# Enigmatisms/Distributed-Machine-Learning-Experiment-Document

Hardware: AMD Instinct MI355X
Metric: samples/sec (whole node) for task3 DDP CNN at 1/2/4/8 MI355X (higher is better)
Workload: dtype bf16; 1 GPU; model=resnet18, global_batch=1024, per_gpu_batch=1024, image_size=224, parallelism=dp1, optimizer=SGD(momentum=0.9), fused flat, ddp=none (dp1: no communication), backend=native, fused_step=False, hip_graph=False, stream_priority=high, sampler=MySampler(partition)

## Files before the change

csrc/stem_fused.hip:

```cpp
#include <type_traits>

#include "common.h"
#include "igemm_common.h"
#include "kernels.h"

namespace dm {

namespace {

constexpr int SCO = 64;
constexpr int SKP = 176;
constexpr int SKH = 192;
constexpr int RING = 13;

typedef short s4v __attribute__((ext_vector_type(4)));
typedef unsigned int nt4 __attribute__((ext_vector_type(4)));
typedef unsigned int nt2 __attribute__((ext_vector_type(2)));
__device__ __forceinline__ s4v tr4(const unsigned char* p) {
  return __builtin_amdgcn_ds_read_tr16_b64_v4i16((__attribute__((address_space(3))) s4v*)p);
}

struct StemGeo {
  int Hin, Win, Hout, Wout, PH, PW;
  int ROWB;
  int SP;
};

struct RawUnit {
  uint4 w;
};

__device__ __forceinline__ void lds_barrier() {
  asm volatile("s_waitcnt lgkmcnt(0)\n\ts_barrier" ::: "memory");
}

__device__ __forceinline__ int ring_of(int iy) { return (iy + 13 * 8) % RING; }

template <int NT, int RU>
struct RawMap {
  int r[RU], k[RU];
  unsigned valid;
  float sc[RU][4], bi[RU][4];
  __device__ __forceinline__ void init(int t, int Win, const float (&nsc)[3], const float (&nbi)[3]) {
    const int upr = 3 * Win / 4;
#pragma unroll
    for (int u = 0; u < RU; ++u) {
      const int e = t + NT * u;
      r[u] = e < 4 * upr ? e / upr : -1;
      k[u] = e - (e / upr) * upr;
#pragma unroll
      for (int j = 0; j < 4; ++j) {
        const int c = (k[u] + j) % 3;
        sc[u][j] = c == 0 ? nsc[0] : c == 1 ? nsc[1] : nsc[2];
        bi[u][j] = c == 0 ? nbi[0] : c == 1 ? nbi[1] : nbi[2];
      }
    }
  }
  template <int DT>
  __device__ __forceinline__ void load(RawUnit (&ru)[RU], const void* img, long long rowbase, int Hin,
                                       int Win, int iy0, int nrows) {
    valid = 0;
#pragma unroll
    for (int u = 0; u < RU; ++u) {
      const int iy = iy0 + r[u];
      const bool ok = r[u] >= 0 && r[u] < nrows && iy >= 0 && iy < Hin;
      valid |= ok ? 1u << u : 0u;
      const int iyc = min(max(iy, 0), Hin - 1);
      const long long off = rowbase + (long long)iyc * Win * 3 + 4LL * (r[u] >= 0 ? k[u] : 0);
      if (DT == 0) {
        ru[u].w = *reinterpret_cast<const uint4*>(reinterpret_cast<const float*>(img) + off);
      } else if (DT == 1) {
        const uint2 w = *reinterpret_cast<const uint2*>(reinterpret_cast<const bf16_t*>(img) + off);
        ru[u].w = make_uint4(w.x, w.y, 0, 0);
      } else {
        ru[u].w = make_uint4(*reinterpret_cast<const uint32_t*>(reinterpret_cast<const uint8_t*>(img) + off), 0, 0, 0);
      }
    }
  }
  template <int DT>
  __device__ __forceinline__ void store(const RawUnit (&ru)[RU], bf16_t* S, int SP, int nrows) const {
#pragma unroll
    for (int u = 0; u < RU; ++u) {
      if (r[u] < 0 || r[u] >= nrows) continue;
      float x[4];
      const uint4 w = ru[u].w;
      if (DT == 0) {
        x[0] = __uint_as_float(w.x); x[1] = __uint_as_float(w.y);
        x[2] = __uint_as_float(w.z); x[3] = __uint_as_float(w.w);
      } else if (DT == 1) {
        x[0] = __uint_as_float(w.x << 16); x[1] = __uint_as_float(w.x & 0xffff0000u);
        x[2] = __uint_as_float(w.y << 16); x[3] = __uint_as_float(w.y & 0xffff0000u);
      } else {
        x[0] = (float)(w.x & 0xff); x[1] = (float)((w.x >> 8) & 0xff);
        x[2] = (float)((w.x >> 16) & 0xff); x[3] = (float)(w.x >> 24);
      }
      const bool ok = (valid >> u) & 1;
#pragma unroll
      for (int j = 0; j < 4; ++j) x[j] = ok ? fmaf(x[j], sc[u][j], bi[u][j]) : 0.f;
      bf16_t* p = S + r[u] * SP + 4 * k[u] + 9;
      p[0] = f2bf(x[0]);
      *reinterpret_cast<uint32_t*>(p + 1) = pack_bf2(x[1], x[2]);
      p[3] = f2bf(x[3]);
    }
  }
};

struct EMap {
  bool act;
  int soff, eoff;
  int part;
  __device__ __forceinline__ void init(int t, int Wout) {
    act = t < 3 * Wout;
    const int ox = t / 3;
    part = t - 3 * ox;
    soff = 6 * ox + 8 * part;
    eoff = 48 * ox + 16 * part;
  }
  __device__ __forceinline__ void build(unsigned char* E, const bf16_t* S, const StemGeo& G, int iy0,
                                        int nrows, int srow0) const {
    if (!act) return;
    if (nrows == 4) build_n<4>(E, S, G, iy0, srow0);
    else if (nrows == 2) build_n<2>(E, S, G, iy0, srow0);
    else for (int q = 0; q < nrows; ++q) build_n<1>(E, S, G, iy0 + q, srow0 + q);
  }
  template <int NR>
  __device__ __forceinline__ void build_n(unsigned char* E, const bf16_t* S, const StemGeo& G,
                                          int iy0, int srow0) const {
    uint32_t w[NR][4];
#pragma unroll
    for (int q = 0; q < NR; ++q) {
      const int sr = min(max(srow0 + q, 0), 3);
      const uint32_t* sp = reinterpret_cast<const uint32_t*>(S + sr * G.SP + soff);
#pragma unroll
      for (int j = 0; j < 4; ++j) w[q][j] = sp[j];
    }
#pragma unroll
    for (int q = 0; q < NR; ++q) {
      const int iy = iy0 + q;
      const bool in = iy >= 0 && iy < G.Hin;
      uint4 v = make_uint4(in ? w[q][0] : 0u, in ? w[q][1] : 0u, in ? w[q][2] : 0u, in ? w[q][3] : 0u);
      if (part == 2) {
        v.z = in ? (v.z & 0xffffu) | 0x3f800000u : 0u;
        v.w = 0;
      }
      *reinterpret_cast<uint4*>(E + ring_of(iy) * G.ROWB + eoff) = v;
    }
  }
};

__host__ __device__ constexpr unsigned wcode(int kh, int kw) { return (unsigned)((2 - kh) << 2 | (2 - kw)); }

__device__ __forceinline__ uint32_t mono2(uint32_t w) {
  const uint32_t s = (w >> 15) & 0x00010001u;
  return w ^ (s * 0x7fffu);
}

__device__ __forceinline__ int yoff(int slot, int px, int c8, int Wout) {
  return ((slot * Wout + px) * 8 + (c8 ^ ((((px >> 1) & 1) << 2) | ((px >> 2) & 3)))) * 16;
}

template <int PF>
__device__ __forceinline__ f32x16 conv_tile(const bf16x8 (&wa)[11], const unsigned char* E,
                                            const int (&rowoff)[7], int pxoff, bool hh) {
  f32x16 acc;
#pragma unroll
  for (int r = 0; r < 16; ++r) acc[r] = 0.f;
  bf16x8 bq[11];
#pragma unroll
  for (int s = 0; s < 11 + PF; ++s) {
    if (s < 11) {
      const int j0 = 2 * s, j1 = 2 * s + 1;
      const int k0 = j0 / 3 > 6 ? 6 : j0 / 3, k1 = j1 / 3 > 6 ? 6 : j1 / 3;
      const int a0 = rowoff[k0] + 16 * (j0 % 3), a1 = rowoff[k1] + 16 * (j1 % 3);
      bq[s] = *reinterpret_cast<const bf16x8*>(E + (hh ? a1 : a0) + pxoff);
    }
    if (s >= PF) acc = __builtin_amdgcn_mfma_f32_32x32x16_bf16(wa[s - PF], bq[s - PF], acc, 0, 0, 0);
  }
  return acc;
}

__device__ __forceinline__ void ring_rows(int (&ro)[7], int iy0, int ROWB) {
  const int r0 = ring_of(iy0);
// ... 355 lines not shown

template <int W>
__device__ __forceinline__ void gram_slot(f32x16 (&acc)[5], const unsigned char* T,
                                          const unsigned char* E, const StemGeo& G, int i,
                                          int slot, int t0, int t1, int lane) {
  constexpr WavePlan P = kPlans[W];
  const int g = lane >> 4, h = g >> 1, i16 = lane & 15, q = i16 >> 2, p = i16 & 3;
  const int oy = 2 * i + slot;
  int boff[4];
#pragma unroll
  for (int b = 0; b < P.nb; ++b) {
    const int k = 32 * P.blk[b] + 16 * (g & 1) + 4 * p;
    int ky = k / 24;
    const int kk = k - 24 * ky;
    if (ky > 6) ky = 6;
    boff[b] = ring_of(2 * oy - 3 + ky) * G.ROWB + (4 * h + q) * 48 + 2 * kk;
  }
  int ta = 0, ta8 = 0;
  if (P.tcb >= 0) {
    const int c8 = 4 * P.tcb + 2 * (g & 1) + (p >> 1);
    ta = yoff(slot, 4 * h + q, c8, G.Wout) + 8 * (p & 1);
    ta8 = yoff(slot, 4 * h + q + 8, c8, G.Wout) + 8 * (p & 1);
  }
  auto load = [&](BwdFrags& F, int t) {
    const int mo = 16 * t;
#pragma unroll
    for (int b = 0; b < P.nb; ++b) {
      const s4v v0 = tr4(E + boff[b] + mo * 48), v1 = tr4(E + boff[b] + (mo + 8) * 48);
      F.xf[b] = (bf16x8){v0[0], v0[1], v0[2], v0[3], v1[0], v1[1], v1[2], v1[3]};
    }
    if (P.tcb >= 0) {
      const s4v v0 = tr4(T + ta + mo * 128), v1 = tr4(T + ta8 + mo * 128);
      F.tf = (bf16x8){v0[0], v0[1], v0[2], v0[3], v1[0], v1[1], v1[2], v1[3]};
    }
  };
  auto mma = [&](const BwdFrags& F) {
#pragma unroll
    for (int j = 0; j < P.nt; ++j)
      acc[j] = __builtin_amdgcn_mfma_f32_32x32x16_bf16(P.kind[j] ? F.tf : F.xf[P.x[j]], F.xf[P.y[j]],
                                                       acc[j], 0, 0, 0);
  };
  for (int t = t0; t < t1; ++t) {
    BwdFrags f;
    load(f, t);
    mma(f);
  }
}

template <int W>
__device__ __forceinline__ void gram_store(const f32x16 (&acc)[5], float* dslab, float* gslab,
                                           int lane) {
  constexpr WavePlan P = kPlans[W];
#pragma unroll
  for (int j = 0; j < P.nt; ++j)
#pragma unroll
    for (int r = 0; r < 16; ++r) {
      const int row = (r & 3) + 8 * (r >> 2) + 4 * (lane >> 5);
      const int col = 32 * P.blk[P.y[j]] + (lane & 31);
      if (P.kind[j])
        dslab[(long long)blockIdx.x * SCO * SKH + (32 * P.tcb + row) * SKH + col] = acc[j][r];
      else
        gslab[(long long)blockIdx.x * GK * GK + (32 * P.blk[P.x[j]] + row) * GK + col] = acc[j][r];
    }
}

template <int W>
__device__ __forceinline__ void gram_zero(f32x16 (&acc)[5]) {
#pragma unroll
  for (int j = 0; j < 5; ++j)
#pragma unroll
    for (int r = 0; r < 16; ++r) acc[j][r] = 0.f;
}

struct StemBwdArgs2 {
  const void* img;
  const long long* idx;
  float nsc[3], nbi[3];
  const bf16_t* wk;
  const bf16_t* pdy;
  const uint8_t* code4;
  float* dslab;
  float* gslab;
  int N, nimg;
  int split;
  StemGeo G;
};

constexpr int PRING = 3;
constexpr int BNT = 1024;
constexpr int BMW = 8;
constexpr int BVT = BNT - 64 * BMW;

template <int DT>
__global__ void __launch_bounds__(BNT, 1) stem_bwd_kernel(StemBwdArgs2 a) {
  extern __shared__ __attribute__((aligned(16))) unsigned char smem[];
  const StemGeo G = a.G;
  const int TB = 2 * G.Wout * 128;
  unsigned char* E = smem;
  unsigned char* T = E + RING * G.ROWB;
  bf16_t* S = reinterpret_cast<bf16_t*>(T + 2 * TB);
  const int PRB = G.PW * SCO;
  bf16_t* Pg = S + 4 * G.SP;
  uint8_t* Pc = reinterpret_cast<uint8_t*>(Pg + PRING * PRB);
  const int tid = threadIdx.x, lane = tid & 63, wid = tid >> 6;
  {
    const int tot16 = (RING * G.ROWB + 2 * TB + 4 * G.SP * 2) / 16;
    for (int e = tid; e < tot16; e += BNT) reinterpret_cast<uint4*>(smem)[e] = make_uint4(0, 0, 0, 0);
  }
  const int nimg = a.N > (int)blockIdx.x ? (a.N - 1 - (int)blockIdx.x) / (int)gridDim.x + 1 : 0;
  const int SPI = G.PH + 2;
  const int nsteps = nimg * SPI;
  auto img_of = [&](int q) { return (int)blockIdx.x + q * (int)gridDim.x; };
  auto img_base = [&](int q) -> long long {
    long long row = a.idx ? a.idx[img_of(q)] : (long long)img_of(q);
    row = row < 0 ? 0 : row >= a.nimg ? a.nimg - 1 : row;
    return row * G.Hin * G.Win * 3;
  };
  if (wid < BMW) {
    f32x16 acc[5];
    gram_zero<0>(acc);
    __syncthreads();
    EMap em;
    em.init(tid, G.Wout);
    auto run = [&](auto wtag) {
      constexpr int W = decltype(wtag)::value;
      for (int st = 0; st <= nsteps; ++st) {
        lds_barrier();
        const int ps = st - 1;
        const int pk = ps >= 0 ? ps % SPI : -1;
        const bool work = ps >= 0 && pk >= 2;
        const unsigned char* Tt = T + (ps & 1) * TB;
        const int nt = G.Wout >> 4, split = min(a.split, 2 * nt);
        if (work) {
          gram_slot<W>(acc, Tt, E, G, pk - 2, 0, 0, min(split, nt), lane);
          if (split > nt) gram_slot<W>(acc, Tt, E, G, pk - 2, 1, 0, split - nt, lane);
        }
        lds_barrier();
        if (work) {
          if (split < nt) gram_slot<W>(acc, Tt, E, G, pk - 2, 0, split, nt, lane);
          gram_slot<W>(acc, Tt, E, G, pk - 2, 1, max(split - nt, 0), nt, lane);
        }
        if (st < nsteps) {
          const int kk = st % SPI;
          if (kk == 1) em.build(E, S, G, -3, 5, -3);
          else if (kk >= 2) em.build(E, S, G, 4 * (kk - 2) + 2, 4, 0);
        }
      }
      gram_store<W>(acc, a.dslab, a.gslab, lane);
    };
    switch (wid) {
      case 0: run(std::integral_constant<int, 0>{}); break;
      case 1: run(std::integral_constant<int, 1>{}); break;
      case 2: run(std::integral_constant<int, 2>{}); break;
      case 3: run(std::integral_constant<int, 3>{}); break;
      case 4: run(std::integral_constant<int, 4>{}); break;
      case 5: run(std::integral_constant<int, 5>{}); break;
      case 6: run(std::integral_constant<int, 6>{}); break;
      default: run(std::integral_constant<int, 7>{}); break;
    }
    return;
  }
  const int vt = tid - 64 * BMW;
  RawMap<BVT, FRU> rm;
  rm.init(vt, G.Win, a.nsc, a.nbi);
  RawUnit ru[FRU];
  const bool pl = vt < G.PW * 8;
  uint4 pg_r;
  uint32_t pc_r;
  bool p_ok = false;
  auto pload = [&](int q, int r) {
    p_ok = pl && r < G.PH;
    const int rc = min(r, G.PH - 1), vc = pl ? vt : 0;
    const long long o = (((long long)img_of(min(q, nimg - 1)) * G.PH + rc) * G.PW) * SCO + vc * 8;
    pg_r = *reinterpret_cast<const uint4*>(a.pdy + o);
    pc_r = *reinterpret_cast<const uint32_t*>(a.code4 + o / 2);
  };
  auto pstore = [&](int r) {
    if (!pl) return;
    const int sl = r % PRING;
    *reinterpret_cast<uint4*>(Pg + sl * PRB + vt * 8) = p_ok ? pg_r : make_uint4(0, 0, 0, 0);
    *reinterpret_cast<uint32_t*>(Pc + (sl * PRB + vt * 8) / 2) = p_ok ? pc_r : 0xffffffffu;
  };
  const int qb = vt >> 3, qc = vt & 7, c0 = qc * 8;
  __syncthreads();
  const bool colok = qb + 1 < G.PW;
  const int ocol0 = qb * SCO + c0, ocol1 = (colok ? qb + 1 : qb) * SCO + c0;
  int toff[4];
#pragma unroll
  for (int pp = 0; pp < 4; ++pp) toff[pp] = yoff(pp >> 1, 2 * qb + (pp & 1), qc, G.Wout);
  uint2 gres[4];
  auto gquad = [&](uint2 (&res)[4], int i, int hf) {
    uint2 qg[4];
    uint32_t qi[4];
    const int sl0 = i % PRING, sl1 = sl0 + 1 == PRING ? 0 : sl0 + 1;
    const bool rowok = i + 1 < G.PH;
#pragma unroll
    for (int w = 0; w < 4; ++w) {
      const int wa = w >> 1, wb = w & 1;
      const int o = (wa ? sl1 : sl0) * PRB + (wb ? ocol1 : ocol0);
      qg[w] = *reinterpret_cast<const uint2*>(Pg + o + 4 * hf);
      const uint32_t c = *reinterpret_cast<const uint16_t*>(Pc + o / 2 + 2 * hf);
      qi[w] = ((wa && !rowok) || (wb && !colok)) ? 0xffffu : c;
    }
#pragma unroll
    for (int pp = 0; pp < 4; ++pp) {
      const int ddy = pp >> 1, ddx = pp & 1;
      float d[4] = {0.f, 0.f, 0.f, 0.f};
#pragma unroll
      for (int w = 0; w < 4; ++w) {
        const int wa = w >> 1, wb = w & 1;
        if ((wa && !ddy) || (wb && !ddx)) continue;
        const uint32_t gw[2] = {qg[w].x, qg[w].y};
        const unsigned code = wcode(ddy ? (wa ? 0 : 2) : 1, ddx ? (wb ? 0 : 2) : 1);
#pragma unroll
        for (int j = 0; j < 4; ++j) {
          const uint32_t g = gw[j >> 1];
          const float gf = __uint_as_float((j & 1) ? (g & 0xffff0000u) : (g << 16));
          d[j] += (qi[w] & (15u << (4 * j))) == (code << (4 * j)) ? gf : 0.f;
        }
      }
      res[pp] = make_uint2(pack_bf2(d[0], d[1]), pack_bf2(d[2], d[3]));
    }
  };


  long long bcur = nimg > 0 ? img_base(0) : 0, bnext = nimg > 1 ? img_base(1) : 0;
  int bq = 0;
  auto base = [&](int qq) {
    if (qq != bq) {
      bcur = bnext;
      bq = qq;
      bnext = qq + 1 < nimg ? img_base(qq + 1) : 0;
    }
    return bcur;
  };
  for (int st = 0; st <= nsteps; ++st) {
    const int q = st / SPI, kk = st - q * SPI;
    lds_barrier();
    if (st < nsteps) {
      if (kk == 0) {
        pload(q, 0);
        pstore(0);
        pload(q, 1);
        pstore(1);
        pload(q, 2);
      } else if (kk == 1) {
        rm.store<DT>(ru, S, G.SP, 2);
      } else {
        const int i = kk - 2;
        pstore(i + 2);
        pload(q, i + 3);
        rm.store<DT>(ru, S, G.SP, 4);
        if (pl) gquad(gres, i, 0);
      }
    }
    lds_barrier();
    if (st < nsteps) {
      if (kk == 0) {
        rm.load<DT>(ru, a.img, base(q), G.Hin, G.Win, 0, 2);
      } else if (kk == 1) {
        rm.load<DT>(ru, a.img, base(q), G.Hin, G.Win, 2, 4);
      } else {
        const int i = kk - 2;
        if (pl) {
          uint2 r1[4];
          gquad(r1, i, 1);
          unsigned char* Tt = T + (st & 1) * TB;
#pragma unroll
          for (int pp = 0; pp < 4; ++pp)
            *reinterpret_cast<uint4*>(Tt + toff[pp]) = make_uint4(gres[pp].x, gres[pp].y, r1[pp].x, r1[pp].y);
        }
        if (i + 1 < G.PH) rm.load<DT>(ru, a.img, base(q), G.Hin, G.Win, 4 * i + 6, 4);
      }
    }
  }
}

__global__ void __launch_bounds__(256) stem_slab_reduce_kernel(const float* __restrict__ dslab,
                                                               const float* __restrict__ gslab,
                                                               int GD, float* __restrict__ dsum,
                                                               float* __restrict__ gsum) {
  const int e = blockIdx.x * 256 + threadIdx.x;
  const int nd = SCO * SKH, ng = GK * GK;
  if (e >= nd + ng) return;
  const float* src = e < nd ? dslab + e : gslab + (e - nd);
  const long long stride = e < nd ? nd : ng;
  float s4[4] = {0.f, 0.f, 0.f, 0.f};
  int gi = 0;
  for (; gi + 4 <= GD; gi += 4)
#pragma unroll
    for (int u = 0; u < 4; ++u) s4[u] += src[(long long)(gi + u) * stride];
  for (; gi < GD; ++gi) s4[0] += src[(long long)gi * stride];
  const float v = (s4[0] + s4[1]) + (s4[2] + s4[3]);
  if (e < nd) dsum[e] = v;
  else gsum[e - nd] = v;
}

__global__ void __launch_bounds__(256) stem_wcombine_kernel(const float* __restrict__ dsum,
                                                            const float* __restrict__ gsum,
                                                            const bf16_t* __restrict__ wk,
                                                            const float* __restrict__ coef,
                                                            float* __restrict__ dw, float beta) {
  __shared__ float wrow[SKP];
  const int co = blockIdx.x, t = threadIdx.x;
  for (int k = t; k < SKP; k += 256) wrow[k] = bf2f(wk[co * SKP + k]);
  __syncthreads();
  if (t >= 147) return;
  const int ky = t / 21, rem = t - 21 * ky, kx = rem / 3, c = rem - 3 * kx;
  const int k = ky * 24 + kx * 3 + c;
  float wg = 0.f;
  for (int j = 0; j < SKP; ++j) {
    const float gv = j <= k ? gsum[j * GK + k] : gsum[k * GK + j];
    wg = fmaf(wrow[j], gv, wg);
  }
  const float colsum = GONE <= k ? gsum[GONE * GK + k] : gsum[k * GK + GONE];
  const float d = coef[co] * dsum[co * SKH + k] + coef[SCO + co] * wg + coef[2 * SCO + co] * colsum;
  float* o = dw + ((co * 3 + c) * 7 + ky) * 7 + kx;
  *o = (beta != 0.f ? beta * *o : 0.f) + d;
}

__global__ void __launch_bounds__(256) stem_pack_weights_kernel(const float* __restrict__ w,
                                                                bf16_t* __restrict__ wk) {
  const int e = blockIdx.x * 256 + threadIdx.x;
  if (e >= SCO * SKP) return;
  const int co = e / SKP, k = e - co * SKP;
  const int ky = k / 24, kk = k - 24 * ky, kx = kk / 3, c = kk - 3 * kx;
  float v = 0.f;
  if (ky < 7 && kk < 21) v = w[((co * 3 + c) * 7 + ky) * 7 + kx];
  wk[e] = f2bf(v);
}

static StemGeo stem_geo(int Hin, int Win) {
  StemGeo G;
  G.Hin = Hin;
  G.Win = Win;
  G.Hout = Hin / 2;
  G.Wout = Win / 2;
  G.PH = G.Hout / 2;
  G.PW = G.Wout / 2;
  G.ROWB = G.Wout * 48;
  G.SP = 3 * Win + 24;
  return G;
}

bool stem_fused_supported(int Hin, int Win) {
  return Hin >= 8 && Hin % 4 == 0 && Win % 32 == 0 && Win <= 224;
}

static size_t fwd_smem(const StemGeo& G) {
  const size_t tiles = (size_t)RING * G.ROWB + (size_t)2 * 2 * G.Wout * 128 + (size_t)2 * 4 * G.SP * 2;
  const size_t red = (size_t)4 * 2 * 16 * 64 * 4;
  return tiles > red ? tiles : red;
}
static size_t bwd_smem(const StemGeo& G) {
  return (size_t)RING * G.ROWB + (size_t)2 * 2 * G.Wout * 128 + (size_t)4 * G.SP * 2 +
         (size_t)PRING * G.PW * SCO * 2 + (size_t)PRING * G.PW * SCO / 2;
}

int stem_fused_grid(int N) {
  static int cus = 0;
  if (!cus) {
    int dev = 0;
    DM_CHECK(hipGetDevice(&dev));
    DM_CHECK(hipDeviceGetAttribute(&cus, hipDeviceAttributeMultiprocessorCount, dev));
  }
  return N < cus ? N : cus;
}

void stem_fwd_fused(const void* img, int dtype, const long long* idx, const float* nsc,
                    const float* nbi, const bf16_t* wk, const float* gamma, bf16_t* pext,
                    uint8_t* code, float* stats, int N, int nimg, int Hin, int Win, int grid,
                    hipStream_t st) {
  StemFwdArgs a;
  a.img = img;
  a.idx = idx;
  for (int c = 0; c < 3; ++c) {
    a.nsc[c] = nsc[c];
    a.nbi[c] = nbi[c];
  }
  a.wk = wk;
  a.gamma = gamma;
  a.pext = pext;
  a.code = code;
  a.stats = stats;
  a.N = N;
  a.nimg = nimg;
  a.G = stem_geo(Hin, Win);
  const size_t sm = fwd_smem(a.G);
#define DM_SF(DT)                                              \
  do {                                                         \
    set_smem_attr(stem_fwd_kernel<DT>, sm);                    \
    stem_fwd_kernel<DT><<<grid, FNT, sm, st>>>(a);             \
  } while (0)
  if (dtype == 0) DM_SF(0);
  else if (dtype == 1) DM_SF(1);
  else DM_SF(2);
#undef DM_SF
  DM_CHECK(hipGetLastError());
}

void stem_pool_apply(const bf16_t* pext, const uint8_t* code, const float* scale,
                     const float* shift, bf16_t* out, uint8_t* code4, long long n, hipStream_t st) {
  const long long n8 = n / 8;
  stem_pool_apply_kernel<<<(unsigned)((n8 + 1023) / 1024), 256, 0, st>>>(
      pext, reinterpret_cast<const uint32_t*>(code), scale, shift, out,
      reinterpret_cast<uint32_t*>(code4), n8);
  DM_CHECK(hipGetLastError());
}

void stem_bwd_fused2(const void* img, int dtype, const long long* idx, const float* nsc,
                     const float* nbi, const bf16_t* wk, const bf16_t* pdy, const uint8_t* code4,
                     float* dslab, float* gslab, int N, int nimg, int Hin, int Win, int grid,
                     hipStream_t st) {
  StemBwdArgs2 a;
  a.img = img;
  a.idx = idx;
  for (int c = 0; c < 3; ++c) {
    a.nsc[c] = nsc[c];
    a.nbi[c] = nbi[c];
  }
  a.wk = wk;
  a.pdy = pdy;
  a.code4 = code4;
  a.dslab = dslab;
  a.gslab = gslab;
  a.N = N;
  a.nimg = nimg;
  a.G = stem_geo(Hin, Win);
  a.split = (2 * (a.G.Wout >> 4) * 5 + 6) / 7;
  const size_t sm = bwd_smem(a.G);
#define DM_SB(DT)                                              \
  do {                                                         \
    set_smem_attr(stem_bwd_kernel<DT>, sm);                    \
    stem_bwd_kernel<DT><<<grid, BNT, sm, st>>>(a);             \
  } while (0)
  if (dtype == 0) DM_SB(0);
  else if (dtype == 1) DM_SB(1);
  else DM_SB(2);
#undef DM_SB
  DM_CHECK(hipGetLastError());
}

void stem_wcombine(const float* dslab, const float* gslab, int GD, const bf16_t* wk,
                   const float* coef, float* sums, float* dw, float beta, hipStream_t st) {
  const int n = SCO * SKH + GK * GK;
  float* dsum = sums;
  float* gsum = sums + SCO * SKH;
  stem_slab_reduce_kernel<<<(n + 255) / 256, 256, 0, st>>>(dslab, gslab, GD, dsum, gsum);
  DM_CHECK(hipGetLastError());
  stem_wcombine_kernel<<<SCO, 256, 0, st>>>(dsum, gsum, wk, coef, dw, beta);
  DM_CHECK(hipGetLastError());
}
int stem_gram_cols() { return GK; }
int stem_sums_len() { return SCO * SKH + GK * GK; }

void stem_pack_weights(const float* w, bf16_t* wk, hipStream_t st) {
  stem_pack_weights_kernel<<<(SCO * SKP + 255) / 256, 256, 0, st>>>(w, wk);
  DM_CHECK(hipGetLastError());
}

int stem_slab_cols() { return SKH; }
int stem_wk_cols() { return SKP; }

}
```

csrc/wgrad_res64.hip:

```cpp
#include "common.h"
#include "conv_geom.h"
#include "igemm_common.h"
#include "kernels.h"

#include <stdexcept>

namespace dm {

namespace {
constexpr int QC = 64;
constexpr int QP = 160;
constexpr int QXS = 66;
constexpr int QDS = 64;
constexpr int QRX = 8;
constexpr int QRD = 6;
constexpr int Q_XROW = QXS * QP;
constexpr int Q_DROW = QDS * QP;
constexpr int Q_X = 0;
constexpr int Q_Z = Q_X + QRX * Q_XROW;
constexpr int Q_D = Q_Z + Q_XROW;
constexpr int Q_SCR = Q_D + QRD * Q_DROW;
constexpr int Q_TAB = Q_SCR;
constexpr int Q_SMEM = Q_TAB + 2 * QC * 4;
constexpr unsigned QOOB = 0x80000000u;

typedef short s4 __attribute__((ext_vector_type(4)));

__device__ __forceinline__ s4 qtr(unsigned lds_byte) {
  return __builtin_amdgcn_ds_read_tr16_b64_v4i16(
      (__attribute__((address_space(3))) s4*)(size_t)lds_byte);
}

template <bool PRE>
__global__ void __launch_bounds__(512, 2) wgrad_res64_kernel(
    const bf16_t* __restrict__ X, const bf16_t* __restrict__ DY, float* __restrict__ slab,
    ConvGeom g, unsigned xbytes, unsigned dybytes, const float* __restrict__ pre_sc,
    const float* __restrict__ pre_sh, int nrows) {
  extern __shared__ __attribute__((aligned(16))) unsigned char smem[];
  const int tid = threadIdx.x, lane = tid & 63;
  const int wid = __builtin_amdgcn_readfirstlane(tid >> 6);
  const int cb = wid & 3, ch = wid >> 2;
  const int W = g.W, H = g.H;

  const int G = gridDim.x, b = blockIdx.x;
  const int per = nrows / G, rem = nrows % G;
  const int r0 = b * per + (b < rem ? b : rem);
  const int r1 = r0 + per + (b < rem ? 1 : 0);

  for (int i = tid; i < Q_SCR / 16; i += 512)
    reinterpret_cast<uint4*>(smem)[i] = make_uint4(0, 0, 0, 0);
  float* tab = reinterpret_cast<float*>(smem + Q_TAB);
  if (PRE && tid < QC) {
    tab[tid] = pre_sc[tid];
    tab[QC + tid] = pre_sh[tid];
  }

  const pi32x4 rsx = prsrc(X, xbytes);
  const pi32x4 rsd = prsrc(DY, dybytes);
  const unsigned lds0 = (unsigned)(size_t)(const __attribute__((address_space(3))) void*)smem;

  const int dslot = lane / 10, dpiece = lane - dslot * 10;
  const bool dlane = lane < 60;
  auto dma_row = [&](const pi32x4& rs, int row, int jj, unsigned lds_row, int rows_total) {
    const int x = 6 * jj + dslot;
    const bool ok = dpiece < 8 && x < W && (unsigned)row < (unsigned)rows_total;
    const unsigned off = ok ? (unsigned)((row * W + x) * 128 + dpiece * 16) : QOOB;
    if (dlane) pdma16(rs, lds_row + (unsigned)(jj * 6 * QP), off);
  };
  const int NR = g.N * H;
  auto xslot = [&](int row) { return (unsigned)(Q_X + ((row % QRX + QRX) % QRX) * Q_XROW); };
  auto dslotb = [&](int row) { return (unsigned)(Q_D + (row % QRD) * Q_DROW); };
  auto batch = [&](int k) __attribute__((always_inline)) {
#pragma unroll
    for (int u = 0; u < 5; ++u) {
      const int j = wid + 8 * u;
      if (j < 20) {
        const int rx = r0 + 2 * k + 1 + j / 10;
        dma_row(rsx, rx, j % 10, lds0 + xslot(rx) + QP, NR);
      } else {
        const int rd = r0 + 2 * k + (j - 20) / 10;
        dma_row(rsd, rd, (j - 20) % 10, lds0 + dslotb(rd), NR);
      }
    }
  };
  auto xonly = [&](int rx) __attribute__((always_inline)) {
#pragma unroll
    for (int u = 0; u < 2; ++u) {
      const int j = wid + 8 * u;
      if (j < 10) dma_row(rsx, rx, j, lds0 + xslot(rx) + QP, NR);
    }
  };
  auto tpiece = [&](int rx, int j) __attribute__((always_inline)) {
    if constexpr (PRE) {
      const int x = 6 * j + dslot;
      if (dlane && dpiece < 8 && x < W) {
        uint4* p = reinterpret_cast<uint4*>(smem + xslot(rx) + QP + j * 6 * QP + lane * 16);
        const float4 s0 = *reinterpret_cast<const float4*>(tab + dpiece * 8);
        const float4 s1 = *reinterpret_cast<const float4*>(tab + dpiece * 8 + 4);
        const float4 h0 = *reinterpret_cast<const float4*>(tab + QC + dpiece * 8);
        const float4 h1 = *reinterpret_cast<const float4*>(tab + QC + dpiece * 8 + 4);
        const float sc[8] = {s0.x, s0.y, s0.z, s0.w, s1.x, s1.y, s1.z, s1.w};
        const float sh[8] = {h0.x, h0.y, h0.z, h0.w, h1.x, h1.y, h1.z, h1.w};
        const uint4 v = *p;
        const uint32_t w[4] = {v.x, v.y, v.z, v.w};
        uint32_t o[4];
#pragma unroll
        for (int q = 0; q < 4; ++q) {
          const float lo = fmaxf(__uint_as_float(w[q] << 16) * sc[2 * q] + sh[2 * q], 0.f);
          const float hi = fmaxf(__uint_as_float(w[q] & 0xffff0000u) * sc[2 * q + 1] + sh[2 * q + 1], 0.f);
          o[q] = pack_bf2(lo, hi);
        }
        *p = make_uint4(o[0], o[1], o[2], o[3]);
      }
    }
  };
  auto xform_batch = [&](int k) __attribute__((always_inline)) {
#pragma unroll
    for (int u = 0; u < 3; ++u) {
      const int j = wid + 8 * u;
      if (j < 20) tpiece(r0 + 2 * k + 1 + j / 10, j % 10);
    }
  };
  auto xform_row = [&](int rx) __attribute__((always_inline)) {
#pragma unroll
    for (int u = 0; u < 2; ++u) {
      const int j = wid + 8 * u;
      if (j < 10) tpiece(rx, j);
    }
  };

  const int grp = lane >> 4, q4 = (lane >> 2) & 3, p4 = lane & 3;
  const int rbase = grp * 4 + q4;
  const unsigned a_lane = (unsigned)(rbase * QP + (ch * 32 + 4 * p4) * 2);
  const unsigned b_lane = (unsigned)(rbase * QP + (cb * 16 + 4 * p4) * 2);

  f32x4 acc[2][9];
#pragma unroll
  for (int i = 0; i < 2; ++i)
#pragma unroll
    for (int t = 0; t < 9; ++t) acc[i][t] = (f32x4){0.f, 0.f, 0.f, 0.f};

  const int niter = (r1 - r0 + 1) / 2;
  if (niter > 0) {
    __syncthreads();
    xonly(r0 - 1);
    xonly(r0);
    batch(0);
    asm volatile("s_waitcnt vmcnt(0)" ::: "memory");
    xform_row(r0 - 1);
    xform_row(r0);
    __syncthreads();
    batch(1);
  }
  for (int it = 0; it < niter; ++it) {
    asm volatile("s_waitcnt vmcnt(5)" ::: "memory");
    xform_batch(it);
    asm volatile("s_waitcnt lgkmcnt(0)\n\ts_barrier" ::: "memory");
    batch(it + 2);

    const int R = r0 + 2 * it;
    const bool two = R + 1 < r1;
    unsigned xb[2][3], ab[2];
#pragma unroll
    for (int ro = 0; ro < 2; ++ro) {
      const int y = (R + ro) % H;
      xb[ro][0] = lds0 + (y > 0 ? xslot(R + ro - 1) : (unsigned)Q_Z) + b_lane;
      xb[ro][1] = lds0 + xslot(R + ro) + b_lane;
      xb[ro][2] = lds0 + (y + 1 < H ? xslot(R + ro + 1) : (unsigned)Q_Z) + b_lane;
      ab[ro] = lds0 + dslotb(R + ro) + a_lane;
    }
    bf16x8 fa[2][2], fb[2][9];
    auto rdk = [&](int set, int ks) __attribute__((always_inline)) {
      const int ro = ks >> 1, kb = ks & 1;
#pragma unroll
      for (int i = 0; i < 2; ++i) {
        const s4 lo = qtr(ab[ro] + (kb * 32) * QP + i * 32);
        const s4 hi = qtr(ab[ro] + (kb * 32 + 16) * QP + i * 32);
        fa[set][i] = (bf16x8){lo[0], lo[1], lo[2], lo[3], hi[0], hi[1], hi[2], hi[3]};
      }
#pragma unroll
      for (int t = 0; t < 9; ++t) {
        const int dyi = t / 3, dxo = t % 3;
        const s4 lo = qtr(xb[ro][dyi] + (kb * 32 + dxo) * QP);
        const s4 hi = qtr(xb[ro][dyi] + (kb * 32 + 16 + dxo) * QP);
        fb[set][t] = (bf16x8){lo[0], lo[1], lo[2], lo[3], hi[0], hi[1], hi[2], hi[3]};
      }
    };
    auto mm = [&](int set) __attribute__((always_inline)) {
#pragma unroll
      for (int t = 0; t < 9; ++t)
#pragma unroll
        for (int i = 0; i < 2; ++i)
          acc[i][t] = __builtin_amdgcn_mfma_f32_16x16x32_bf16(fa[set][i], fb[set][t], acc[i][t], 0, 0, 0);
    };
    rdk(0, 0);
    rdk(1, 1);
    __builtin_amdgcn_sched_barrier(0);
    mm(0);
    __builtin_amdgcn_sched_barrier(0);
    if (two) {
      rdk(0, 2);
      __builtin_amdgcn_sched_barrier(0);
      mm(1);
      __builtin_amdgcn_sched_barrier(0);
      rdk(1, 3);
      __builtin_amdgcn_sched_barrier(0);
      mm(0);
      __builtin_amdgcn_sched_barrier(0);
      mm(1);
    } else {
      mm(1);
    }
  }
  asm volatile("s_waitcnt vmcnt(0)" ::: "memory");

  float* out = slab + (long long)b * QC * 9 * QC;
  const int c = cb * 16 + (lane & 15);
#pragma unroll
  for (int i = 0; i < 2; ++i)
#pragma unroll
    for (int t = 0; t < 9; ++t)
#pragma unroll
      for (int rr = 0; rr < 4; ++rr) {
        const int co = ch * 32 + i * 16 + (lane >> 4) * 4 + rr;
        out[co * 9 * QC + t * QC + c] = acc[i][t][rr];
      }
}
}

bool wgrad_res64_supported(const ConvGeom& g) {
  if (g.C != QC || g.Ncols != QC || g.K != 9 * QC) return false;
  if (g.isy != 1 || g.isx != 1 || g.Hg != g.H || g.Wg != g.W || g.W > 60) return false;
  if (g.nth != 3 || g.ntw != 3 || g.dy0 != -1 || g.dys != 1 || g.dx0 != -1 || g.dxs != 1) return false;
  if (g.kh0 != 0 || g.khs != 1 || g.kw0 != 0 || g.kws != 1 || g.KW != 3) return false;
  return (long long)g.N * g.H * g.W * QC * 2 < (1LL << 31);
}

void wgrad_res64(const bf16_t* X, const bf16_t* DY, float* slab, const ConvGeom& g, int S,
                 hipStream_t st, const float* pre_sc, const float* pre_sh) {
  if (!wgrad_res64_supported(g)) throw std::runtime_error("wgrad_res64: unsupported geometry");
  const int nrows = g.N * g.H;
  if (S < 1 || S > nrows) throw std::runtime_error("wgrad_res64: S must be in [1, N*H]");
  const unsigned bytes = (unsigned)((long long)g.N * g.H * g.W * QC * 2);
  auto k = pre_sc ? wgrad_res64_kernel<true> : wgrad_res64_kernel<false>;
  set_smem_attr(k, Q_SMEM);
  k<<<S, 512, Q_SMEM, st>>>(X, DY, slab, g, bytes, bytes, pre_sc, pre_sh, nrows);
  DM_CHECK(hipGetLastError());
}

}
```

Measured before the change: 57170 samples/s.

## Restructure stem backward pipeline to one barrier per step with register pool rows

Reorganizes the stem backward kernel's producer loop so each pipeline step uses a single LDS barrier instead of two. It double-buffers the S staging buffer and keeps pooled-gradient and code rows in registers (PoolRow rotation) instead of an LDS ring. Raw image loads are prefetched one step ahead, and the MFMA waves' gram work is no longer split across two barrier phases. The aim is to cut barrier stalls and LDS traffic and to raise occupancy headroom, at the cost of more registers per producer thread and slightly changed load/store ordering.

```diff
diff --git a/csrc/stem_bwd_lds.h b/csrc/stem_bwd_lds.h
--- /dev/null
+++ b/csrc/stem_bwd_lds.h
@@ -0,0 +1,37 @@
+#pragma once
+
+#include <cstddef>
+
+namespace dm {
+
+constexpr int kStemRing = 13;
+constexpr int kStemLdsMax = 160 * 1024;
+constexpr int kStemMaxWin = 224;
+
+constexpr bool stem_size_supported(int Hin, int Win) {
+  return Hin >= 8 && Hin % 4 == 0 && Win % 32 == 0 && Win <= kStemMaxWin;
+}
+
+struct StemBwdLds {
+  int e_off, e_bytes;
+  int t_off, t_bytes;
+  int s_off, s_bytes;
+  int total;
+  constexpr int tile_bytes() const { return t_bytes / 2; }
+  constexpr int sbuf_bytes() const { return s_bytes / 2; }
+};
+
+constexpr StemBwdLds stem_bwd_lds(int Win) {
+  const int Wout = Win / 2, SP = 3 * Win + 24;
+  StemBwdLds L{};
+  L.e_off = 0;
+  L.e_bytes = kStemRing * Wout * 48;
+  L.t_off = L.e_off + L.e_bytes;
+  L.t_bytes = 2 * 2 * Wout * 128;
+  L.s_off = L.t_off + L.t_bytes;
+  L.s_bytes = 2 * 4 * SP * 2;
+  L.total = L.s_off + L.s_bytes;
+  return L;
+}
+
+}
diff --git a/csrc/stem_fused.hip b/csrc/stem_fused.hip
--- a/csrc/stem_fused.hip
+++ b/csrc/stem_fused.hip
@@ -3,6 +3,7 @@
 #include "common.h"
 #include "igemm_common.h"
 #include "kernels.h"
+#include "stem_bwd_lds.h"
 
 namespace dm {
 
@@ -36,20 +37,25 @@
 
 __device__ __forceinline__ int ring_of(int iy) { return (iy + 13 * 8) % RING; }
 
-template <int NT, int RU>
+template <int NT, int RU, bool KEEP = true>
 struct RawMap {
   int r[RU], k[RU];
   unsigned valid;
-  float sc[RU][4], bi[RU][4];
+  float sc[KEEP ? RU : 1][4], bi[KEEP ? RU : 1][4];
+  float n3[2][3];
   __device__ __forceinline__ void init(int t, int Win, const float (&nsc)[3], const float (&nbi)[3]) {
     const int upr = 3 * Win / 4;
+    if (!KEEP) {
+#pragma unroll
+      for (int c = 0; c < 3; ++c) n3[0][c] = nsc[c], n3[1][c] = nbi[c];
+    }
 #pragma unroll
     for (int u = 0; u < RU; ++u) {
       const int e = t + NT * u;
       r[u] = e < 4 * upr ? e / upr : -1;
       k[u] = e - (e / upr) * upr;
 #pragma unroll
-      for (int j = 0; j < 4; ++j) {
+      for (int j = 0; j < (KEEP ? 4 : 0); ++j) {
         const int c = (k[u] + j) % 3;
         sc[u][j] = c == 0 ? nsc[0] : c == 1 ? nsc[1] : nsc[2];
         bi[u][j] = c == 0 ? nbi[0] : c == 1 ? nbi[1] : nbi[2];
@@ -66,7 +72,12 @@
       const bool ok = r[u] >= 0 && r[u] < nrows && iy >= 0 && iy < Hin;
       valid |= ok ? 1u << u : 0u;
       const int iyc = min(max(iy, 0), Hin - 1);
-      const long long off = rowbase + (long long)iyc * Win * 3 + 4LL * (r[u] >= 0 ? k[u] : 0);
+      long long off = rowbase + (long long)iyc * Win * 3 + 4LL * (r[u] >= 0 ? k[u] : 0);
+      if (!KEEP) {
+        int ku = r[u] >= 0 ? k[u] : 0;
+        asm volatile("" : "+v"(ku));
+        off = rowbase + (long long)iyc * Win * 3 + 4LL * ku;
+      }
       if (DT == 0) {
         ru[u].w = *reinterpret_cast<const uint4*>(reinterpret_cast<const float*>(img) + off);
       } else if (DT == 1) {
@@ -82,6 +93,8 @@
 #pragma unroll
     for (int u = 0; u < RU; ++u) {
       if (r[u] < 0 || r[u] >= nrows) continue;
+      int ks = k[u];
+      if (!KEEP) asm volatile("" : "+v"(ks));
       float x[4];
       const uint4 w = ru[u].w;
       if (DT == 0) {
@@ -95,9 +108,21 @@
         x[2] = (float)((w.x >> 16) & 0xff); x[3] = (float)(w.x >> 24);
       }
       const bool ok = (valid >> u) & 1;
-#pragma unroll
-      for (int j = 0; j < 4; ++j) x[j] = ok ? fmaf(x[j], sc[u][j], bi[u][j]) : 0.f;
-      bf16_t* p = S + r[u] * SP + 4 * k[u] + 9;
+      if (KEEP) {
+#pragma unroll
+        for (int j = 0; j < 4; ++j) x[j] = ok ? fmaf(x[j], sc[u][j], bi[u][j]) : 0.f;
+      } else {
+        const int c0 = ks % 3;
+        float s3[3], b3[3];
+#pragma unroll
+        for (int j = 0; j < 3; ++j) {
+          s3[j] = c0 == 0 ? n3[0][j] : c0 == 1 ? n3[0][(j + 1) % 3] : n3[0][(j + 2) % 3];
+          b3[j] = c0 == 0 ? n3[1][j] : c0 == 1 ? n3[1][(j + 1) % 3] : n3[1][(j + 2) % 3];
+        }
+#pragma unroll
+        for (int j = 0; j < 4; ++j) x[j] = ok ? fmaf(x[j], s3[j % 3], b3[j % 3]) : 0.f;
+      }
+      bf16_t* p = S + r[u] * SP + 4 * ks + 9;
       p[0] = f2bf(x[0]);
       *reinterpret_cast<uint32_t*>(p + 1) = pack_bf2(x[1], x[2]);
       p[3] = f2bf(x[3]);
@@ -619,31 +644,31 @@
   float* dslab;
   float* gslab;
   int N, nimg;
-  int split;
   StemGeo G;
 };
 
-constexpr int PRING = 3;
 constexpr int BNT = 1024;
 constexpr int BMW = 8;
 constexpr int BVT = BNT - 64 * BMW;
+static_assert(RING == kStemRing, "stem_bwd_lds.h sizes the E ring");
+
+struct PoolRow {
+  uint4 g0, g1;
+  uint32_t c0, c1;
+};
 
 template <int DT>
 __global__ void __launch_bounds__(BNT, 1) stem_bwd_kernel(StemBwdArgs2 a) {
   extern __shared__ __attribute__((aligned(16))) unsigned char smem[];
   const StemGeo G = a.G;
-  const int TB = 2 * G.Wout * 128;
-  unsigned char* E = smem;
-  unsigned char* T = E + RING * G.ROWB;
-  bf16_t* S = reinterpret_cast<bf16_t*>(T + 2 * TB);
-  const int PRB = G.PW * SCO;
-  bf16_t* Pg = S + 4 * G.SP;
-  uint8_t* Pc = reinterpret_cast<uint8_t*>(Pg + PRING * PRB);
+  const StemBwdLds L = stem_bwd_lds(G.Win);
+  const int TB = L.tile_bytes();
+  unsigned char* E = smem + L.e_off;
+  unsigned char* T = smem + L.t_off;
+  bf16_t* S = reinterpret_cast<bf16_t*>(smem + L.s_off);
+  const int SB = 4 * G.SP;
   const int tid = threadIdx.x, lane = tid & 63, wid = tid >> 6;
-  {
-    const int tot16 = (RING * G.ROWB + 2 * TB + 4 * G.SP * 2) / 16;
-    for (int e = tid; e < tot16; e += BNT) reinterpret_cast<uint4*>(smem)[e] = make_uint4(0, 0, 0, 0);
-  }
+  for (int e = tid; e < L.total / 16; e += BNT) reinterpret_cast<uint4*>(smem)[e] = make_uint4(0, 0, 0, 0);
   const int nimg = a.N > (int)blockIdx.x ? (a.N - 1 - (int)blockIdx.x) / (int)gridDim.x + 1 : 0;
   const int SPI = G.PH + 2;
   const int nsteps = nimg * SPI;
@@ -661,26 +686,21 @@
     em.init(tid, G.Wout);
     auto run = [&](auto wtag) {
       constexpr int W = decltype(wtag)::value;
+      const int nt = G.Wout >> 4;
       for (int st = 0; st <= nsteps; ++st) {
         lds_barrier();
         const int ps = st - 1;
         const int pk = ps >= 0 ? ps % SPI : -1;
-        const bool work = ps >= 0 && pk >= 2;
-        const unsigned char* Tt = T + (ps & 1) * TB;
-        const int nt = G.Wout >> 4, split = min(a.split, 2 * nt);
-        if (work) {
-          gram_slot<W>(acc, Tt, E, G, pk - 2, 0, 0, min(split, nt), lane);
-          if (split > nt) gram_slot<W>(acc, Tt, E, G, pk - 2, 1, 0, split - nt, lane);
-        }
-        lds_barrier();
-        if (work) {
-          if (split < nt) gram_slot<W>(acc, Tt, E, G, pk - 2, 0, split, nt, lane);
-          gram_slot<W>(acc, Tt, E, G, pk - 2, 1, max(split - nt, 0), nt, lane);
+        if (ps >= 0 && pk >= 2) {
+          const unsigned char* Tt = T + (ps & 1) * TB;
+          gram_slot<W>(acc, Tt, E, G, pk - 2, 0, 0, nt, lane);
+          gram_slot<W>(acc, Tt, E, G, pk - 2, 1, 0, nt, lane);
         }
         if (st < nsteps) {
           const int kk = st % SPI;
-          if (kk == 1) em.build(E, S, G, -3, 5, -3);
-          else if (kk >= 2) em.build(E, S, G, 4 * (kk - 2) + 2, 4, 0);
+          const bf16_t* Sp = S + ((st - 1) & 1) * SB;
+          if (kk == 1) em.build(E, Sp, G, -3, 5, -3);
+          else if (kk >= 2) em.build(E, Sp, G, 4 * (kk - 2) + 2, 4, 0);
         }
       }
       gram_store<W>(acc, a.dslab, a.gslab, lane);
@@ -698,46 +718,39 @@
     return;
   }
   const int vt = tid - 64 * BMW;
-  RawMap<BVT, FRU> rm;
+  RawMap<BVT, FRU, false> rm;
   rm.init(vt, G.Win, a.nsc, a.nbi);
   RawUnit ru[FRU];
   const bool pl = vt < G.PW * 8;
-  uint4 pg_r;
-  uint32_t pc_r;
-  bool p_ok = false;
-  auto pload = [&](int q, int r) {
-    p_ok = pl && r < G.PH;
-    const int rc = min(r, G.PH - 1), vc = pl ? vt : 0;
-    const long long o = (((long long)img_of(min(q, nimg - 1)) * G.PH + rc) * G.PW) * SCO + vc * 8;
-    pg_r = *reinterpret_cast<const uint4*>(a.pdy + o);
-    pc_r = *reinterpret_cast<const uint32_t*>(a.code4 + o / 2);
-  };
-  auto pstore = [&](int r) {
-    if (!pl) return;
-    const int sl = r % PRING;
-    *reinterpret_cast<uint4*>(Pg + sl * PRB + vt * 8) = p_ok ? pg_r : make_uint4(0, 0, 0, 0);
-    *reinterpret_cast<uint32_t*>(Pc + (sl * PRB + vt * 8) / 2) = p_ok ? pc_r : 0xffffffffu;
-  };
-  const int qb = vt >> 3, qc = vt & 7, c0 = qc * 8;
+  const int qb = vt >> 3, qc = vt & 7;
+  const bool colok = qb + 1 < G.PW;
+  PoolRow p0 = {}, p1 = {}, pn = {};
+  auto pload = [&](PoolRow& P, int q, int r) {
+    int vc = vt;
+    asm volatile("" : "+v"(vc));
+    const int nx = (vc >> 3) + 1 < G.PW ? SCO : 0;
+    vc = vc < G.PW * 8 ? vc : 0;
+    const int rc = min(r, G.PH - 1);
+    const long long o = (((long long)img_of(q) * G.PH + rc) * G.PW) * SCO + vc * 8;
+    P.g0 = *reinterpret_cast<const uint4*>(a.pdy + o);
+    P.c0 = *reinterpret_cast<const uint32_t*>(a.code4 + o / 2);
+    P.g1 = *reinterpret_cast<const uint4*>(a.pdy + o + nx);
+    P.c1 = *reinterpret_cast<const uint32_t*>(a.code4 + (o + nx) / 2);
+  };
   __syncthreads();
-  const bool colok = qb + 1 < G.PW;
-  const int ocol0 = qb * SCO + c0, ocol1 = (colok ? qb + 1 : qb) * SCO + c0;
-  int toff[4];
-#pragma unroll
-  for (int pp = 0; pp < 4; ++pp) toff[pp] = yoff(pp >> 1, 2 * qb + (pp & 1), qc, G.Wout);
-  uint2 gres[4];
-  auto gquad = [&](uint2 (&res)[4], int i, int hf) {
+  const int toff[2] = {yoff(0, 2 * qb, qc, G.Wout), yoff(0, 2 * qb + 1, qc, G.Wout)};
+  auto gquad = [&](uint2 (&res)[4], const PoolRow& r0, const PoolRow& r1, int i, int hf) {
     uint2 qg[4];
     uint32_t qi[4];
-    const int sl0 = i % PRING, sl1 = sl0 + 1 == PRING ? 0 : sl0 + 1;
     const bool rowok = i + 1 < G.PH;
 #pragma unroll
     for (int w = 0; w < 4; ++w) {
       const int wa = w >> 1, wb = w & 1;
-      const int o = (wa ? sl1 : sl0) * PRB + (wb ? ocol1 : ocol0);
-      qg[w] = *reinterpret_cast<const uint2*>(Pg + o + 4 * hf);
-      const uint32_t c = *reinterpret_cast<const uint16_t*>(Pc + o / 2 + 2 * hf);
-      qi[w] = ((wa && !rowok) || (wb && !colok)) ? 0xffffu : c;
+      const PoolRow& R = wa ? r1 : r0;
+      const uint4 g = wb ? R.g1 : R.g0;
+      qg[w] = hf ? make_uint2(g.z, g.w) : make_uint2(g.x, g.y);
+      const uint32_t c = wb ? R.c1 : R.c0;
+      qi[w] = ((wa && !rowok) || (wb && !colok)) ? 0xffffu : hf ? c >> 16 : c & 0xffffu;
     }
 #pragma unroll
     for (int pp = 0; pp < 4; ++pp) {
@@ -759,7 +772,6 @@
       res[pp] = make_uint2(pack_bf2(d[0], d[1]), pack_bf2(d[2], d[3]));
     }
   };
-
 
   long long bcur = nimg > 0 ? img_base(0) : 0, bnext = nimg > 1 ? img_base(1) : 0;
   int bq = 0;
@@ -771,44 +783,30 @@
     }
     return bcur;
   };
+  if (nimg > 0) rm.load<DT>(ru, a.img, base(0), G.Hin, G.Win, 0, 2);
   for (int st = 0; st <= nsteps; ++st) {
     const int q = st / SPI, kk = st - q * SPI;
     lds_barrier();
-    if (st < nsteps) {
-      if (kk == 0) {
-        pload(q, 0);
-        pstore(0);
-        pload(q, 1);
-        pstore(1);
-        pload(q, 2);
-      } else if (kk == 1) {
-        rm.store<DT>(ru, S, G.SP, 2);
-      } else {
-        const int i = kk - 2;
-        pstore(i + 2);
-        pload(q, i + 3);
-        rm.store<DT>(ru, S, G.SP, 4);
-        if (pl) gquad(gres, i, 0);
-      }
-    }
-    lds_barrier();
-    if (st < nsteps) {
-      if (kk == 0) {
-        rm.load<DT>(ru, a.img, base(q), G.Hin, G.Win, 0, 2);
-      } else if (kk == 1) {
-        rm.load<DT>(ru, a.img, base(q), G.Hin, G.Win, 2, 4);
-      } else {
-        const int i = kk - 2;
-        if (pl) {
-          uint2 r1[4];
-          gquad(r1, i, 1);
-          unsigned char* Tt = T + (st & 1) * TB;
-#pragma unroll
-          for (int pp = 0; pp < 4; ++pp)
-            *reinterpret_cast<uint4*>(Tt + toff[pp]) = make_uint4(gres[pp].x, gres[pp].y, r1[pp].x, r1[pp].y);
-        }
-        if (i + 1 < G.PH) rm.load<DT>(ru, a.img, base(q), G.Hin, G.Win, 4 * i + 6, 4);
-      }
+    if (st == nsteps) break;
+    const int nst = kk == 0 ? 2 : kk <= G.PH ? 4 : 0;
+    if (nst) rm.store<DT>(ru, S + (st & 1) * SB, G.SP, nst);
+    if (kk >= 1) {
+      p0 = p1;
+      p1 = pn;
+    }
+    if (kk + 1 <= G.PH) rm.load<DT>(ru, a.img, base(q), G.Hin, G.Win, 4 * kk + 2, 4);
+    else if (kk == G.PH + 1 && q + 1 < nimg) rm.load<DT>(ru, a.img, base(q + 1), G.Hin, G.Win, 0, 2);
+    pload(pn, q, kk);
+    if (kk >= 2 && pl) {
+      const int i = kk - 2;
+      uint2 r0[4], r1[4];
+      gquad(r0, p0, p1, i, 0);
+      gquad(r1, p0, p1, i, 1);
+      unsigned char* Tt = T + (st & 1) * TB;
+#pragma unroll
+      for (int pp = 0; pp < 4; ++pp)
+        *reinterpret_cast<uint4*>(Tt + (pp >> 1) * (TB / 2) + toff[pp & 1]) =
+            make_uint4(r0[pp].x, r0[pp].y, r1[pp].x, r1[pp].y);
     }
   }
 }
@@ -881,7 +879,7 @@
 }
 
 bool stem_fused_supported(int Hin, int Win) {
-  return Hin >= 8 && Hin % 4 == 0 && Win % 32 == 0 && Win <= 224;
+  return stem_size_supported(Hin, Win);
 }
 
 static size_t fwd_smem(const StemGeo& G) {
@@ -889,10 +887,7 @@
   const size_t red = (size_t)4 * 2 * 16 * 64 * 4;
   return tiles > red ? tiles : red;
 }
-static size_t bwd_smem(const StemGeo& G) {
-  return (size_t)RING * G.ROWB + (size_t)2 * 2 * G.Wout * 128 + (size_t)4 * G.SP * 2 +
-         (size_t)PRING * G.PW * SCO * 2 + (size_t)PRING * G.PW * SCO / 2;
-}
+static size_t bwd_smem(const StemGeo& G) { return (size_t)stem_bwd_lds(G.Win).total; }
 
 int stem_fused_grid(int N) {
   static int cus = 0;
@@ -964,7 +959,6 @@
   a.N = N;
   a.nimg = nimg;
   a.G = stem_geo(Hin, Win);
-  a.split = (2 * (a.G.Wout >> 4) * 5 + 6) / 7;
   const size_t sm = bwd_smem(a.G);
 #define DM_SB(DT)                                              \
   do {                                                         \
```

Result: no change. 56980 samples/s (-0.3%).

## Interleave next-batch BN-ReLU prologue transform with MFMA in res64 wgrad

Applied to the files above, without the earlier changes.

The wgrad kernel for 64-channel 3x3 convs applies a fused BN+ReLU to the input rows staged in LDS. That transform used to run as a separate phase before each compute step; it now runs one batch ahead and is split into pieces interleaved between MFMA groups using scheduling barriers. The per-channel scale and shift are kept in registers instead of an LDS table, and the bf16 packing uses a vector convert. This is meant to hide the transform's VALU and LDS work behind matrix ops, at the cost of more register pressure and a more fragile instruction schedule.

```diff
diff --git a/csrc/wgrad_res64.hip b/csrc/wgrad_res64.hip
--- a/csrc/wgrad_res64.hip
+++ b/csrc/wgrad_res64.hip
@@ -19,12 +19,17 @@
 constexpr int Q_X = 0;
 constexpr int Q_Z = Q_X + QRX * Q_XROW;
 constexpr int Q_D = Q_Z + Q_XROW;
-constexpr int Q_SCR = Q_D + QRD * Q_DROW;
-constexpr int Q_TAB = Q_SCR;
-constexpr int Q_SMEM = Q_TAB + 2 * QC * 4;
+constexpr int Q_SMEM = Q_D + QRD * Q_DROW;
 constexpr unsigned QOOB = 0x80000000u;
 
 typedef short s4 __attribute__((ext_vector_type(4)));
+
+typedef float qf2 __attribute__((ext_vector_type(2)));
+typedef __bf16 qb2 __attribute__((ext_vector_type(2)));
+
+__device__ __forceinline__ uint32_t qpack(float lo, float hi) {
+  return __builtin_bit_cast(uint32_t, __builtin_convertvector((qf2){lo, hi}, qb2));
+}
 
 __device__ __forceinline__ s4 qtr(unsigned lds_byte) {
   return __builtin_amdgcn_ds_read_tr16_b64_v4i16(
@@ -47,13 +52,8 @@
   const int r0 = b * per + (b < rem ? b : rem);
   const int r1 = r0 + per + (b < rem ? 1 : 0);
 
-  for (int i = tid; i < Q_SCR / 16; i += 512)
+  for (int i = tid; i < Q_SMEM / 16; i += 512)
     reinterpret_cast<uint4*>(smem)[i] = make_uint4(0, 0, 0, 0);
-  float* tab = reinterpret_cast<float*>(smem + Q_TAB);
-  if (PRE && tid < QC) {
-    tab[tid] = pre_sc[tid];
-    tab[QC + tid] = pre_sh[tid];
-  }
 
   const pi32x4 rsx = prsrc(X, xbytes);
   const pi32x4 rsd = prsrc(DY, dybytes);
@@ -90,28 +90,44 @@
       if (j < 10) dma_row(rsx, rx, j, lds0 + xslot(rx) + QP, NR);
     }
   };
+  float psc[8], psh[8];
+  if constexpr (PRE) {
+    const int c0 = (dpiece & 7) * 8;
+    const float4 s0 = *reinterpret_cast<const float4*>(pre_sc + c0);
+    const float4 s1 = *reinterpret_cast<const float4*>(pre_sc + c0 + 4);
+    const float4 h0 = *reinterpret_cast<const float4*>(pre_sh + c0);
+    const float4 h1 = *reinterpret_cast<const float4*>(pre_sh + c0 + 4);
+    psc[0] = s0.x; psc[1] = s0.y; psc[2] = s0.z; psc[3] = s0.w;
+    psc[4] = s1.x; psc[5] = s1.y; psc[6] = s1.z; psc[7] = s1.w;
+    psh[0] = h0.x; psh[1] = h0.y; psh[2] = h0.z; psh[3] = h0.w;
+    psh[4] = h1.x; psh[5] = h1.y; psh[6] = h1.z; psh[7] = h1.w;
+#pragma unroll
+    for (int i = 0; i < 8; ++i) asm volatile("" : "+v"(psc[i]), "+v"(psh[i]));
+  }
+  auto tguard = [&](int rx, int j, bool live, bool& ok) __attribute__((always_inline)) {
+    const int x = 6 * j + dslot;
+    ok = (int)live & (int)dlane & (int)(dpiece < 8) & (int)(x < W) &
+         (int)((unsigned)rx < (unsigned)NR);
+    return xslot(rx) + (unsigned)(QP + j * 6 * QP + ((int)live & (int)dlane ? lane : 8) * 16);
+  };
+  auto tpair = [&](uint32_t w, int q, bool ok) __attribute__((always_inline)) {
+    const float lo = fmaxf(__uint_as_float(w << 16) * psc[2 * q] + psh[2 * q], 0.f);
+    const float hi = fmaxf(__uint_as_float(w & 0xffff0000u) * psc[2 * q + 1] + psh[2 * q + 1], 0.f);
+    return ok ? qpack(lo, hi) : w;
+  };
   auto tpiece = [&](int rx, int j) __attribute__((always_inline)) {
     if constexpr (PRE) {
-      const int x = 6 * j + dslot;
-      if (dlane && dpiece < 8 && x < W) {
-        uint4* p = reinterpret_cast<uint4*>(smem + xslot(rx) + QP + j * 6 * QP + lane * 16);
-        const float4 s0 = *reinterpret_cast<const float4*>(tab + dpiece * 8);
-        const float4 s1 = *reinterpret_cast<const float4*>(tab + dpiece * 8 + 4);
-        const float4 h0 = *reinterpret_cast<const float4*>(tab + QC + dpiece * 8);
-        const float4 h1 = *reinterpret_cast<const float4*>(tab + QC + dpiece * 8 + 4);
-        const float sc[8] = {s0.x, s0.y, s0.z, s0.w, s1.x, s1.y, s1.z, s1.w};
-        const float sh[8] = {h0.x, h0.y, h0.z, h0.w, h1.x, h1.y, h1.z, h1.w};
-        const uint4 v = *p;
-        const uint32_t w[4] = {v.x, v.y, v.z, v.w};
-        uint32_t o[4];
-#pragma unroll
-        for (int q = 0; q < 4; ++q) {
-          const float lo = fmaxf(__uint_as_float(w[q] << 16) * sc[2 * q] + sh[2 * q], 0.f);
-          const float hi = fmaxf(__uint_as_float(w[q] & 0xffff0000u) * sc[2 * q + 1] + sh[2 * q + 1], 0.f);
-          o[q] = pack_bf2(lo, hi);
-        }
-        *p = make_uint4(o[0], o[1], o[2], o[3]);
-      }
+      bool ok;
+      uint4* p = reinterpret_cast<uint4*>(smem + tguard(rx, j, true, ok));
+      const uint4 v = *p;
+      *p = make_uint4(tpair(v.x, 0, ok), tpair(v.y, 1, ok), tpair(v.z, 2, ok), tpair(v.w, 3, ok));
+    }
+  };
+  auto xform_row = [&](int rx) __attribute__((always_inline)) {
+#pragma unroll
+    for (int u = 0; u < 2; ++u) {
+      const int j = wid + 8 * u;
+      if (j < 10) tpiece(rx, j);
     }
   };
   auto xform_batch = [&](int k) __attribute__((always_inline)) {
@@ -119,13 +135,6 @@
     for (int u = 0; u < 3; ++u) {
       const int j = wid + 8 * u;
       if (j < 20) tpiece(r0 + 2 * k + 1 + j / 10, j % 10);
-    }
-  };
-  auto xform_row = [&](int rx) __attribute__((always_inline)) {
-#pragma unroll
-    for (int u = 0; u < 2; ++u) {
-      const int j = wid + 8 * u;
-      if (j < 10) tpiece(rx, j);
     }
   };
 
@@ -149,12 +158,12 @@
     asm volatile("s_waitcnt vmcnt(0)" ::: "memory");
     xform_row(r0 - 1);
     xform_row(r0);
+    if constexpr (PRE) xform_batch(0);
     __syncthreads();
     batch(1);
   }
   for (int it = 0; it < niter; ++it) {
-    asm volatile("s_waitcnt vmcnt(5)" ::: "memory");
-    xform_batch(it);
+    if constexpr (!PRE) asm volatile("s_waitcnt vmcnt(5)" ::: "memory");
     asm volatile("s_waitcnt lgkmcnt(0)\n\ts_barrier" ::: "memory");
     batch(it + 2);
 
@@ -186,28 +195,69 @@
         fb[set][t] = (bf16x8){lo[0], lo[1], lo[2], lo[3], hi[0], hi[1], hi[2], hi[3]};
       }
     };
-    auto mm = [&](int set) __attribute__((always_inline)) {
-#pragma unroll
-      for (int t = 0; t < 9; ++t)
-#pragma unroll
-        for (int i = 0; i < 2; ++i)
-          acc[i][t] = __builtin_amdgcn_mfma_f32_16x16x32_bf16(fa[set][i], fb[set][t], acc[i][t], 0, 0, 0);
+    auto mf = [&](int set, int n0, int n1) __attribute__((always_inline)) {
+#pragma unroll
+      for (int n = n0; n < n1; ++n)
+        acc[n & 1][n >> 1] = __builtin_amdgcn_mfma_f32_16x16x32_bf16(
+            fa[set][n & 1], fb[set][n >> 1], acc[n & 1][n >> 1], 0, 0, 0);
     };
+    auto mm = [&](int set) __attribute__((always_inline)) { mf(set, 0, 18); };
     rdk(0, 0);
     rdk(1, 1);
     __builtin_amdgcn_sched_barrier(0);
     mm(0);
     __builtin_amdgcn_sched_barrier(0);
     if (two) {
+      unsigned tp[3];
+      bool tok[3];
+      if constexpr (PRE) {
+        asm volatile("s_waitcnt vmcnt(5)" ::: "memory");
+        const bool next = it + 1 < niter;
+#pragma unroll
+        for (int u = 0; u < 3; ++u) {
+          const int j = wid + 8 * u;
+          const bool live = (int)next & (int)(j < 20);
+          const int jj = j < 20 ? j : wid;
+          tp[u] = tguard(R + 3 + jj / 10, jj % 10, live, tok[u]);
+        }
+      }
+      uint4 tv[3];
+      auto tread = [&](int u) __attribute__((always_inline)) {
+        if constexpr (PRE) tv[u] = *reinterpret_cast<const uint4*>(smem + tp[u]);
+      };
+      auto mmx = [&](int set, int u) __attribute__((always_inline)) {
+        if constexpr (PRE) {
+          const uint32_t w[4] = {tv[u].x, tv[u].y, tv[u].z, tv[u].w};
+          uint32_t o[4];
+          mf(set, 0, 6);
+#pragma unroll
+          for (int q = 0; q < 4; ++q) {
+            __builtin_amdgcn_sched_barrier(0);
+            mf(set, 6 + 3 * q, 9 + 3 * q);
+            o[q] = tpair(w[q], q, tok[u]);
+#pragma unroll
+            for (int k = 0; k < 3; ++k) {
+              __builtin_amdgcn_sched_group_barrier(0x008, 1, 0);
+              __builtin_amdgcn_sched_group_barrier(0x002, 3, 0);
+            }
+          }
+          *reinterpret_cast<uint4*>(smem + tp[u]) = make_uint4(o[0], o[1], o[2], o[3]);
+        } else {
+          mm(set);
+        }
+      };
+      tread(0);
       rdk(0, 2);
       __builtin_amdgcn_sched_barrier(0);
-      mm(1);
+      mmx(1, 0);
       __builtin_amdgcn_sched_barrier(0);
+      tread(1);
+      tread(2);
       rdk(1, 3);
       __builtin_amdgcn_sched_barrier(0);
-      mm(0);
+      mmx(0, 1);
       __builtin_amdgcn_sched_barrier(0);
-      mm(1);
+      mmx(1, 2);
     } else {
       mm(1);
     }
```

New measurement: 57120 samples/s before, 56760 samples/s after. No clear change (-0.6%).
